# yuki-koyama/sequential-line-search

Hardware: AMD Instinct MI355X
Metric: GP-fit+acq-max step time (ms) and candidate-evals/sec at N=8192 D=64 (higher is better)
Workload: dtype f64

## Files before the change

sequential-line-search_amd/csrc/gemm_f64.hpp:

```cpp
#pragma once
#include <hip/hip_runtime.h>

namespace slsk {

typedef double d4_t __attribute__((ext_vector_type(4)));
typedef double d2_t __attribute__((ext_vector_type(2)));

constexpr int GEMM_BM = 128;
constexpr int GEMM_BN = 128;
constexpr int GEMM_BK = 16;
constexpr int GEMM_THREADS = 256;
constexpr int GEMM_LDS_MC_LD = 144;
constexpr int GEMM_LDS_KC_LD = 18;
constexpr int GEMM_LDS_TILE = 16 * 144;
constexpr int GEMM_LDS_BYTES = 4 * GEMM_LDS_TILE * 8;

struct Acc {
    d4_t v[4][4];
    __device__ __forceinline__ void zero() {
#pragma unroll
        for (int i = 0; i < 4; ++i)
#pragma unroll
            for (int j = 0; j < 4; ++j) v[i][j] = d4_t{0.0, 0.0, 0.0, 0.0};
    }
// ... 10 lines not shown
        const int idx = tid + 256 * i;
        if (!KC) {
            const int k = idx >> 6, m2 = idx & 63;
            s.r[i] = *reinterpret_cast<const d2_t*>(P + (long)(2 * m2) + (long)(k0 + k) * ld);
        } else {
            const int m = idx >> 3, k2 = idx & 7;
            s.r[i] = *reinterpret_cast<const d2_t*>(P + (long)(k0 + 2 * k2) + (long)m * ld);
        }
    }
}

template <bool KC>
__device__ __forceinline__ void stage_store(const Stage& s, double* lds, int tid) {
#pragma unroll
    for (int i = 0; i < 4; ++i) {
        const int idx = tid + 256 * i;
        if (!KC) {
            const int k = idx >> 6, m2 = idx & 63;
            *reinterpret_cast<d2_t*>(lds + k * GEMM_LDS_MC_LD + 2 * m2) = s.r[i];
        } else {
            const int m = idx >> 3, k2 = idx & 7;
            *reinterpret_cast<d2_t*>(lds + m * GEMM_LDS_KC_LD + 2 * k2) = s.r[i];
        }
    }
}

template <bool KC>
__device__ __forceinline__ double frag_read(const double* lds, int mbase, int kk, int lane) {
    if (!KC)
        return lds[(4 * kk + (lane >> 4)) * GEMM_LDS_MC_LD + mbase + (lane & 15)];
    else
        return lds[(mbase + (lane & 15)) * GEMM_LDS_KC_LD + 4 * kk + (lane >> 4)];
}

__device__ __forceinline__ void slab_row_to_lds(const double* g, double* l) {
    __builtin_amdgcn_global_load_lds((const __attribute__((address_space(1))) void*)g, (__attribute__((address_space(3))) void*)l, 16, 0,
                                     0);
}

__device__ __forceinline__ void slab_row_to_lds_sc1(const double* g, double* l) {
    __builtin_amdgcn_global_load_lds((const __attribute__((address_space(1))) void*)g, (__attribute__((address_space(3))) void*)l, 16, 0,
                                     16);
}

__device__ __forceinline__ void slab_row_to_lds_saddr(const double* srow, unsigned lane_off, unsigned lds_byte_addr) {
    asm volatile("s_mov_b32 m0, %2\n\ts_nop 0\n\tglobal_load_lds_dwordx4 %0, %1" ::"v"(lane_off), "s"(srow), "s"(lds_byte_addr)
                 : "memory", "m0");
}

template <int N>
__device__ __forceinline__ void ring_wait_barrier() {
    asm volatile("s_waitcnt vmcnt(%0) lgkmcnt(0)\n\ts_barrier" ::"n"(N) : "memory");
}

template <int NJ, int CUR>
__device__ __forceinline__ void mc_slab(Acc& acc, double (&f0)[4 + NJ], double (&f1)[4 + NJ], const double* Arow, const double* Brow,
                                        long lda, long ldb, unsigned lane_off, unsigned lds_base, const double* lds, int cur_rt,
                                        int nxt_rt, int wave, int wm, int wn, int lane) {
    const int cur_off = CUR < 0 ? cur_rt : CUR * 2 * GEMM_LDS_TILE;
    const int nxt_off = CUR < 0 ? nxt_rt : (1 - CUR) * 2 * GEMM_LDS_TILE;
    auto issue = [&](int l) {
        const int r = l & 3;
        const double* g = l < 4 ? Arow + (long)r * lda : Brow + (long)r * ldb;
        const unsigned d = lds_base + 8u * (unsigned)(nxt_off + (l < 4 ? 0 : GEMM_LDS_TILE) + (4 * wave + r) * GEMM_LDS_MC_LD);
        slab_row_to_lds_saddr(g, lane_off, d);
    };
    auto read = [&](double (&f)[4 + NJ], int bufoff, int kk) {
#pragma unroll
        for (int i = 0; i < 4; ++i) f[i] = frag_read<false>(lds + bufoff, wm + 16 * i, kk, lane);
#pragma unroll
        for (int j = 0; j < NJ; ++j) f[4 + j] = frag_read<false>(lds + bufoff + GEMM_LDS_TILE, wn + 16 * j, kk, lane);
    };
#pragma unroll
    for (int kk = 0; kk < 4; ++kk) {
        double(&f)[4 + NJ] = (kk & 1) ? f1 : f0;
        double(&g)[4 + NJ] = (kk & 1) ? f0 : f1;
#pragma unroll
        for (int i = 0; i < 4; ++i) {
#pragma unroll
            for (int j = 0; j < NJ; ++j) {
                acc.v[i][j] = __builtin_amdgcn_mfma_f64_16x16x4f64(f[4 + j], f[i], acc.v[i][j], 0, 0, 0);
                const int m = (kk * 4 + i) * NJ + j + 1;
                if ((m & 1) == 0 && m <= 16) {
                    __builtin_amdgcn_sched_barrier(0);
                    issue(m / 2 - 1);
                    __builtin_amdgcn_sched_barrier(0);
                }
            }
            if (kk < 3 && i == 2) {
                __builtin_amdgcn_sched_barrier(0);
                read(g, cur_off, kk + 1);
                __builtin_amdgcn_sched_barrier(0);
            }
            if (kk == 3 && i == 1) {
                __builtin_amdgcn_sched_barrier(0);
                ring_wait_barrier<0>();
                read(g, nxt_off, 0);
                __builtin_amdgcn_sched_barrier(0);
            }
        }
    }
}

template <int NJ = 4, bool EVEN = false>
__device__ __forceinline__ void gemm_tile_mc(Acc& acc, const double* __restrict__ A, long lda, const double* __restrict__ B, long ldb,
                                             int kb, int ke, double* lds, int nhalf = 0) {
    if (kb >= ke) return;
    const int tid = threadIdx.x, lane = tid & 63;
    const int wave = __builtin_amdgcn_readfirstlane(tid >> 6);
    const int wm = (wave & 1) * 64;
    const int wn = NJ == 4 ? (wave >> 1) * 64 : 64 * nhalf + (wave >> 1) * 32;
    const unsigned lane_off = 16u * lane;
    const unsigned lds_base = (unsigned)(unsigned long long)(__attribute__((address_space(3))) double*)lds;
    const double* A0 = A + (long)(kb + 4 * wave) * lda;
    const double* B0 = B + (long)(kb + 4 * wave) * ldb;
#pragma unroll
    for (int r = 0; r < 4; ++r) {
        slab_row_to_lds_saddr(A0 + (long)r * lda, lane_off, lds_base + 8u * (unsigned)((4 * wave + r) * GEMM_LDS_MC_LD));
        slab_row_to_lds_saddr(B0 + (long)r * ldb, lane_off, lds_base + 8u * (unsigned)(GEMM_LDS_TILE + (4 * wave + r) * GEMM_LDS_MC_LD));
    }
    ring_wait_barrier<0>();
    double f0[4 + NJ], f1[4 + NJ];
#pragma unroll
    for (int i = 0; i < 4; ++i) f0[i] = frag_read<false>(lds, wm + 16 * i, 0, lane);
#pragma unroll
    for (int j = 0; j < NJ; ++j) f0[4 + j] = frag_read<false>(lds + GEMM_LDS_TILE, wn + 16 * j, 0, lane);
    const int nslab = (ke - kb) / GEMM_BK;
    const double* Arow = A0;
    const double* Brow = B0;
    if constexpr (EVEN) {
        for (int s = 0; s < nslab; s += 2) {
            Arow += (long)GEMM_BK * lda;
            Brow += (long)GEMM_BK * ldb;
            mc_slab<NJ, 0>(acc, f0, f1, Arow, Brow, lda, ldb, lane_off, lds_base, lds, 0, 0, wave, wm, wn, lane);
            const bool last = s + 2 == nslab;
            Arow = last ? A0 : Arow + (long)GEMM_BK * lda;
            Brow = last ? B0 : Brow + (long)GEMM_BK * ldb;
            mc_slab<NJ, 1>(acc, f0, f1, Arow, Brow, lda, ldb, lane_off, lds_base, lds, 0, 0, wave, wm, wn, lane);
        }
    } else {
        int cur = 0;
        for (int s = 0; s < nslab; ++s) {
            const bool last = s + 1 == nslab;
            Arow = last ? A0 : Arow + (long)GEMM_BK * lda;
            Brow = last ? B0 : Brow + (long)GEMM_BK * ldb;
            const int nxt = cur ^ (2 * GEMM_LDS_TILE);
            mc_slab<NJ, -1>(acc, f0, f1, Arow, Brow, lda, ldb, lane_off, lds_base, lds, cur, nxt, wave, wm, wn, lane);
            cur = nxt;
        }
    }
    ring_wait_barrier<0>();
}

template <bool A_KC, bool B_KC, int NJ = 4, bool EVEN = false>
__device__ __forceinline__ void gemm_tile(Acc& acc, const double* __restrict__ A, long lda,
                                          const double* __restrict__ B, long ldb, int kb, int ke, double* lds, int nhalf = 0) {
    if constexpr (!A_KC && !B_KC) {
        gemm_tile_mc<NJ, EVEN>(acc, A, lda, B, ldb, kb, ke, lds, nhalf);
    } else {
        static_assert(NJ == 4, "half tiles exist for the M-contiguous form only");
        const int tid = threadIdx.x;
        const int lane = tid & 63;
        const int wave = tid >> 6;
        const int wm = (wave & 1) * 64;
        const int wn = (wave >> 1) * 64;
        if (kb >= ke) return;
        Stage sa, sb;
        stage_load<A_KC>(sa, A, lda, kb, tid);
        stage_load<B_KC>(sb, B, ldb, kb, tid);
        stage_store<A_KC>(sa, lds, tid);
        stage_store<B_KC>(sb, lds + GEMM_LDS_TILE, tid);
        __syncthreads();
        int cur = 0;
        for (int k0 = kb; k0 < ke; k0 += GEMM_BK) {
            const bool more = (k0 + GEMM_BK) < ke;
            if (more) {
                stage_load<A_KC>(sa, A, lda, k0 + GEMM_BK, tid);
                stage_load<B_KC>(sb, B, ldb, k0 + GEMM_BK, tid);
            }
            const double* la = lds + cur;
            const double* lb = lds + cur + GEMM_LDS_TILE;
#pragma unroll
            for (int kk = 0; kk < 4; ++kk) {
                double af[4], bf[4];
#pragma unroll
                for (int i = 0; i < 4; ++i) af[i] = frag_read<A_KC>(la, wm + 16 * i, kk, lane);
#pragma unroll
                for (int j = 0; j < 4; ++j) bf[j] = frag_read<B_KC>(lb, wn + 16 * j, kk, lane);
#pragma unroll
                for (int i = 0; i < 4; ++i)
#pragma unroll
                    for (int j = 0; j < 4; ++j)
                        acc.v[i][j] = __builtin_amdgcn_mfma_f64_16x16x4f64(bf[j], af[i], acc.v[i][j], 0, 0, 0);
            }
            const int nxt = cur ^ (2 * GEMM_LDS_TILE);
            if (more) {
                stage_store<A_KC>(sa, lds + nxt, tid);
                stage_store<B_KC>(sb, lds + nxt + GEMM_LDS_TILE, tid);
            }
            __syncthreads();
            cur = nxt;
        }
    }
}

constexpr int GEMM_N64_LDS_B = 64 * GEMM_LDS_KC_LD;
constexpr int GEMM_N64_LDS_BUF = GEMM_LDS_TILE + GEMM_N64_LDS_B;
constexpr int GEMM_N64_LDS_BYTES = 2 * GEMM_N64_LDS_BUF * 8;

struct Acc64 {
    d4_t v[2][4];
    __device__ __forceinline__ void zero() {
#pragma unroll
        for (int i = 0; i < 2; ++i)
#pragma unroll
            for (int j = 0; j < 4; ++j) v[i][j] = d4_t{0.0, 0.0, 0.0, 0.0};
    }
};

template <int A_LD>
constexpr int gemm_n64_lds_bytes() {
    return 2 * (16 * A_LD + GEMM_N64_LDS_B) * 8;
}
template <bool A_KC = false, int A_LD = GEMM_LDS_MC_LD>
__device__ __forceinline__ void gemm_tile_n64(Acc64& acc, const double* __restrict__ A, long lda,
                                              const double* __restrict__ B, long ldb, int kb, int ke, double* lds) {
    static_assert(!A_KC || A_LD == GEMM_LDS_MC_LD, "the K-contiguous image has its own padding");
    constexpr int A_SLAB = 16 * A_LD;
    constexpr int BUF = A_SLAB + GEMM_N64_LDS_B;
    const int tid = threadIdx.x;
    const int lane = tid & 63;
    const int wm = (tid >> 6) * 32;
    if (kb >= ke) return;
    Stage sa;
    d2_t sbr[2];
    auto load_b = [&](int k0) {
#pragma unroll
        for (int i = 0; i < 2; ++i) {
            const int idx = tid + 256 * i;
            const int n = idx >> 3, k2 = idx & 7;
            sbr[i] = *reinterpret_cast<const d2_t*>(B + (long)(k0 + 2 * k2) + (long)n * ldb);
        }
    };
    auto store_b = [&](double* l) {
#pragma unroll
        for (int i = 0; i < 2; ++i) {
            const int idx = tid + 256 * i;
            const int n = idx >> 3, k2 = idx & 7;
            *reinterpret_cast<d2_t*>(l + n * GEMM_LDS_KC_LD + 2 * k2) = sbr[i];
        }
    };
    constexpr bool DIRECT_A = !A_KC;
    const int wave_u = __builtin_amdgcn_readfirstlane(tid >> 6);
    auto issue_a = [&](int k0, int bufoff) {
#pragma unroll
        for (int r = 0; r < 4; ++r) {
            const int row = 4 * wave_u + r;
            slab_row_to_lds(A + 2 * lane + (long)(k0 + row) * lda, lds + bufoff + row * A_LD);
        }
    };
    if (DIRECT_A) issue_a(kb, 0);
    else stage_load<A_KC>(sa, A, lda, kb, tid);
    load_b(kb);
    if (DIRECT_A) asm volatile("s_waitcnt vmcnt(0)" ::: "memory");
    else stage_store<A_KC>(sa, lds, tid);
    store_b(lds + A_SLAB);
    __syncthreads();
    int cur = 0;
    for (int k0 = kb; k0 < ke; k0 += GEMM_BK) {
        const bool more = (k0 + GEMM_BK) < ke;
        if (more) {
            if (DIRECT_A) issue_a(k0 + GEMM_BK, cur ^ BUF);
            else stage_load<A_KC>(sa, A, lda, k0 + GEMM_BK, tid);
            load_b(k0 + GEMM_BK);
        }
        const double* la = lds + cur;
        const double* lb = lds + cur + A_SLAB;
#pragma unroll
        for (int kk = 0; kk < 4; ++kk) {
            double af[2], bf[4];
#pragma unroll
            for (int i = 0; i < 2; ++i)
                af[i] = A_KC ? frag_read<true>(la, wm + 16 * i, kk, lane)
                             : la[(4 * kk + (lane >> 4)) * A_LD + wm + 16 * i + (lane & 15)];
#pragma unroll
            for (int j = 0; j < 4; ++j) bf[j] = frag_read<true>(lb, 16 * j, kk, lane);
#pragma unroll
            for (int i = 0; i < 2; ++i)
#pragma unroll
                for (int j = 0; j < 4; ++j)
                    acc.v[i][j] = __builtin_amdgcn_mfma_f64_16x16x4f64(bf[j], af[i], acc.v[i][j], 0, 0, 0);
        }
        const int nxt = cur ^ BUF;
        if (more) {
            if (!DIRECT_A) stage_store<A_KC>(sa, lds + nxt, tid);
            store_b(lds + nxt + A_SLAB);
        }
        if (DIRECT_A) asm volatile("s_waitcnt vmcnt(0)" ::: "memory");
        __syncthreads();
        cur = nxt;
    }
}

__device__ __forceinline__ int acc_m(int i) {
    const int lane = threadIdx.x & 63, wave = threadIdx.x >> 6;
    return (wave & 1) * 64 + 16 * i + (lane & 15);
}
__device__ __forceinline__ int acc_n(int j, int r) {
    const int lane = threadIdx.x & 63, wave = threadIdx.x >> 6;
    return (wave >> 1) * 64 + 16 * j + (lane >> 4) + 4 * r;
}

template <bool HEAVY = false, class F>
__device__ __forceinline__ void acc_tile_by_columns(const Acc& acc, double* lds, F&& f) {
    const int lane = threadIdx.x & 63, wave = __builtin_amdgcn_readfirstlane(threadIdx.x >> 6);
#pragma unroll
    for (int half = 0; half < 2; ++half) {
        __syncthreads();
        if ((wave >> 1) == half) {
#pragma unroll
            for (int i = 0; i < 4; ++i)
#pragma unroll
                for (int j = 0; j < 4; ++j)
#pragma unroll
                    for (int r = 0; r < 4; ++r)
                        lds[(16 * j + (lane >> 4) + 4 * r) * GEMM_LDS_MC_LD + (wave & 1) * 64 + 16 * i + (lane & 15)] = acc.v[i][j][r];
        }
        __syncthreads();
        if constexpr (HEAVY) {
#pragma unroll 2
            for (int q = 0; q < 16; ++q) {
                const int c = wave + 4 * q;
                const d2_t v = *reinterpret_cast<const d2_t*>(lds + c * GEMM_LDS_MC_LD + 2 * lane);
                f(64 * half + c, 2 * lane, v);
            }
        } else {
#pragma unroll
            for (int q = 0; q < 16; ++q) {
                const int c = wave + 4 * q;
                const d2_t v = *reinterpret_cast<const d2_t*>(lds + c * GEMM_LDS_MC_LD + 2 * lane);
                f(64 * half + c, 2 * lane, v);
            }
        }
    }
}

__device__ __forceinline__ int xcd_remap(int b, int nwg) {
    const int q = nwg >> 3, r = nwg & 7;
    const int xcd = b & 7, within = b >> 3;
    const int base = (xcd < r) ? xcd * (q + 1) : r * (q + 1) + (xcd - r) * q;
    return base + within;
}

}
```

sequential-line-search_amd/csrc/kernels_acq.hip:

```cpp
#include <cstdlib>

#include "gemm_f64.hpp"
#include "kernels.hpp"
#include "../../include/sls_hip.h"

namespace slsk {

template <bool MATERN, bool HALF>
__device__ __forceinline__ void acq_tile(int t, int nhalf, int ntm, int ntn, const double* __restrict__ Ks, const double* __restrict__ Cs,
                                         long ldk, const double* __restrict__ Kinv, int Np, double* __restrict__ P,
                                         double* __restrict__ kw_part, double* __restrict__ cw_part, double* lds) {
    const int GM = 8;
    const int gsz = GM * ntn;
    const int g = t / gsz, w = t % gsz;
    const int gm = min(GM, ntm - g * GM);
    const int tm = g * GM + (w % gm), tn = w / gm;
    const int m0 = tm * GEMM_BM, n0 = tn * GEMM_BN;
    Acc acc;
    acc.zero();
    gemm_tile<false, false, HALF ? 2 : 4, true>(acc, Ks + m0, ldk, Kinv + n0, (long)Np, 0, Np, lds, nhalf);
    const int lane = threadIdx.x & 63, wave = threadIdx.x >> 6;
    constexpr int NJ = HALF ? 2 : 4;
    const int nbase = HALF ? 64 * nhalf + (wave >> 1) * 32 : (wave >> 1) * 64;
    double* red = lds;
    double* ex = lds + 1024;
    if (HALF && (wave >> 1) == 1) __syncthreads();
    double skw[4], scw[4];
#pragma unroll
    for (int i = 0; i < 4; ++i) {
        const long gm_ = m0 + acc_m(i);
        double pk = 0.0, pc = 0.0;
        if (HALF && (wave >> 1) == 1) {
            pk = ex[((0 * 2 + (wave & 1)) * 4 + i) * 64 + lane];
            pc = ex[((1 * 2 + (wave & 1)) * 4 + i) * 64 + lane];
        }
        double kv[NJ][4], cv[NJ][4];
#pragma unroll
        for (int j = 0; j < NJ; ++j)
#pragma unroll
            for (int r = 0; r < 4; ++r) {
                const long off = gm_ + (long)(n0 + nbase + 16 * j + (lane >> 4) + 4 * r) * ldk;
                kv[j][r] = Ks[off];
                if (MATERN) cv[j][r] = Cs[off];
            }
#pragma unroll
        for (int j = 0; j < NJ; ++j)
#pragma unroll
            for (int r = 0; r < 4; ++r) {
                const long off = gm_ + (long)(n0 + nbase + 16 * j + (lane >> 4) + 4 * r) * ldk;
                const double wv = acc.v[i][j][r];
                const double k = kv[j][r];
                const double c = MATERN ? cv[j][r] : k;
                const double p = c * wv;
                P[off] = p;
                pc += p;
                if (MATERN) pk += k * wv;
            }
        if (HALF && (wave >> 1) == 0) {
            ex[((0 * 2 + (wave & 1)) * 4 + i) * 64 + lane] = pk;
            ex[((1 * 2 + (wave & 1)) * 4 + i) * 64 + lane] = pc;
        }
        scw[i] = pc;
        skw[i] = MATERN ? pk : pc;
    }
    if (HALF && (wave >> 1) == 0) __syncthreads();
#pragma unroll
    for (int i = 0; i < 4; ++i) {
        skw[i] += __shfl_xor(skw[i], 16);
        skw[i] += __shfl_xor(skw[i], 32);
        scw[i] += __shfl_xor(scw[i], 16);
        scw[i] += __shfl_xor(scw[i], 32);
    }
    if (lane < 16 && (!HALF || (wave >> 1) == 1)) {
#pragma unroll
        for (int i = 0; i < 4; ++i) {
            const int ml = (wave & 1) * 64 + 16 * i + lane;
            const int slot = HALF ? 0 : (wave >> 1);
            red[(slot * 2 + 0) * 128 + ml] = skw[i];
            red[(slot * 2 + 1) * 128 + ml] = scw[i];
        }
    }
    __syncthreads();
    if (threadIdx.x < 128) {
        const int ml = threadIdx.x;
        if (HALF) {
            kw_part[(long)(2 * tn + nhalf) * ldk + m0 + ml] = red[0 * 128 + ml];
            cw_part[(long)(2 * tn + nhalf) * ldk + m0 + ml] = red[1 * 128 + ml];
        } else {
            kw_part[(long)(2 * tn + 0) * ldk + m0 + ml] = red[0 * 128 + ml] + red[2 * 128 + ml];
            cw_part[(long)(2 * tn + 0) * ldk + m0 + ml] = red[1 * 128 + ml] + red[3 * 128 + ml];
        }
    }
}

template <bool MATERN>
__global__ __launch_bounds__(256, 1) void acq_gemm_kernel(const double* __restrict__ Ks, const double* __restrict__ Cs, long ldk,
                                                          int Sp, const double* __restrict__ Kinv, int Np,
                                                          double* __restrict__ P, double* __restrict__ kw_part,
                                                          double* __restrict__ cw_part, int* __restrict__ sync,
                                                          int phase, int ntiles, int prio, int gate_every, int nx) {
    extern __shared__ __attribute__((aligned(16))) char smem[];
    double* lds = reinterpret_cast<double*>(smem);
    const int ntm = Sp / GEMM_BM, ntn = Np / GEMM_BN;
    if (sync == nullptr) {
        acq_tile<MATERN, false>(xcd_remap(blockIdx.x, ntiles), 0, ntm, ntn, Ks, Cs, ldk, Kinv, Np, P, kw_part, cw_part, lds);
        return;
    }
    const int xcd = blockIdx.x % nx, slot = blockIdx.x / nx, slots = gridDim.x / nx;
    const int nchunks = (ntiles + slots - 1) / slots;
    const int half = slots >> 1;
    const int grp = phase > 0 ? (slot >= half ? 1 : 0) : 0;
    if (prio && slot >= half) __builtin_amdgcn_s_setprio(1);
    int* gate = sync + 2 * xcd + grp;
    const int per_gen = phase > 0 ? half : slots;
    if (grp == 1) {
        if (threadIdx.x == 0) {
            const long long t0 = wall_clock64();
            while (wall_clock64() - t0 < phase) __builtin_amdgcn_s_sleep(16);
        }
        __syncthreads();
    }
    int gen = 0;
    for (int c = xcd; c < nchunks; c += nx, ++gen) {
        if (gen > 0 && phase >= 0 && gen % gate_every == 0) {
            if (threadIdx.x == 0) {
                const int target = per_gen * gen;
                const long long t0 = wall_clock64();
                while (__hip_atomic_load(gate, __ATOMIC_RELAXED, __HIP_MEMORY_SCOPE_AGENT) < target &&
                       wall_clock64() - t0 < 20000)
                    __builtin_amdgcn_s_sleep(16);
            }
            __syncthreads();
        }
        const int t = c * slots + slot;
        if (t < ntiles) acq_tile<MATERN, false>(t, 0, ntm, ntn, Ks, Cs, ldk, Kinv, Np, P, kw_part, cw_part, lds);
        __syncthreads();
        if (threadIdx.x == 0) __hip_atomic_fetch_add(gate, 1, __ATOMIC_RELAXED, __HIP_MEMORY_SCOPE_AGENT);
    }
}

template <bool MATERN>
__global__ __launch_bounds__(256, 1) void acq_gemm_half_kernel(const double* __restrict__ Ks, const double* __restrict__ Cs, long ldk,
                                                               int Sp, const double* __restrict__ Kinv, int Np,
                                                               double* __restrict__ P, double* __restrict__ kw_part,
                                                               double* __restrict__ cw_part, int tail_first) {
    extern __shared__ __attribute__((aligned(16))) char smem[];
    double* lds = reinterpret_cast<double*>(smem);
    const int u = xcd_remap(blockIdx.x, gridDim.x);
    acq_tile<MATERN, true>(tail_first + (u >> 1), u & 1, Sp / GEMM_BM, Np / GEMM_BN, Ks, Cs, ldk, Kinv, Np, P, kw_part, cw_part, lds);
}

int launch_acq_gemm(hipStream_t s, const double* Ks, const double* Cs, long ldk, int Sp, const double* Kinv, int Np, double* P,
                    double* kw_part, double* cw_part, int* sync) {
    const int nt = (Sp / GEMM_BM) * (Np / GEMM_BN);
    const int persist_env = (int)tune(TUNE_PERSIST, 1);
    const int phase = (int)tune(TUNE_GATE_PHASE, tune(TUNE_ACQ_WG_PER_CU, 1) == 2 ? 2000 : 0);
    const int gate_every = std::max(1, (int)tune(TUNE_GATE_EVERY, tune(TUNE_ACQ_WG_PER_CU, 1) == 2 ? 1 : 16));
    const int prio = 0;
    const int wg_per_cu = tune(TUNE_ACQ_WG_PER_CU, 1) == 2 ? 2 : 1;
    const ChipGeometry chip = chip_geometry();
    const int cap = chip.n_cu * wg_per_cu;
    const int nx = (chip.n_xcd <= 8 && cap % chip.n_xcd == 0) ? chip.n_xcd : 1;
    const int lds_bytes = wg_per_cu == 1 ? 96 * 1024 : GEMM_LDS_BYTES;
    ensure_dyn_lds((const void*)acq_gemm_kernel<false>, lds_bytes);
    ensure_dyn_lds((const void*)acq_gemm_kernel<true>, lds_bytes);
    ensure_dyn_lds((const void*)acq_gemm_half_kernel<false>, lds_bytes);
    ensure_dyn_lds((const void*)acq_gemm_half_kernel<true>, lds_bytes);
    const bool persist = persist_env && sync && nt >= 2 * cap && Np >= 2048;
    const int phase_k = persist_env == 2 ? -1 : phase;
    const bool tail_ok = tune_on(TUNE_TAIL_SPLIT);
    const int rem = nt % cap;
    const int tail = (tail_ok && rem > 0 && rem <= cap / 2) ? rem : 0;
    const int nmain = nt - tail;
    int* sy = nullptr;
    int grid = nmain;
    if (persist && nmain >= 2 * cap) {
        (void)hipMemsetAsync(sync, 0, 16 * sizeof(int), s);
        sy = sync;
        grid = cap;
    }
    const bool matern = Cs != Ks;
    if (nmain > 0) {
        if (matern)
            hipLaunchKernelGGL(acq_gemm_kernel<true>, dim3(grid), dim3(GEMM_THREADS), lds_bytes, s, Ks, Cs, ldk, Sp, Kinv, Np, P,
                               kw_part, cw_part, sy, phase_k, nmain, prio, gate_every, nx);
        else
            hipLaunchKernelGGL(acq_gemm_kernel<false>, dim3(grid), dim3(GEMM_THREADS), lds_bytes, s, Ks, Cs, ldk, Sp, Kinv, Np, P,
                               kw_part, cw_part, sy, phase_k, nmain, prio, gate_every, nx);
    }
    if (tail > 0) {
        if (matern)
            hipLaunchKernelGGL(acq_gemm_half_kernel<true>, dim3(2 * tail), dim3(GEMM_THREADS), lds_bytes, s, Ks, Cs, ldk, Sp, Kinv,
                               Np, P, kw_part, cw_part, nmain);
        else
            hipLaunchKernelGGL(acq_gemm_half_kernel<false>, dim3(2 * tail), dim3(GEMM_THREADS), lds_bytes, s, Ks, Cs, ldk, Sp, Kinv,
                               Np, P, kw_part, cw_part, nmain);
    }
    return nmain;
}

__device__ __forceinline__ void var_tile(int tm, int tn, const double* __restrict__ Ks, long ldk, const double* __restrict__ Linv,
                                         int Np, double* __restrict__ kw_part, double* __restrict__ cw_part, double* lds) {
    const int m0 = tm * GEMM_BM, n0 = tn * GEMM_BN;
    Acc acc;
    acc.zero();
    gemm_tile<false, false, 4, true>(acc, Ks + m0, ldk, Linv + n0, (long)Np, 0, GEMM_BN * (tn + 1), lds);
    const int lane = threadIdx.x & 63, wave = threadIdx.x >> 6;
    double sv[4];
#pragma unroll
    for (int i = 0; i < 4; ++i) {
        double p = 0.0;
#pragma unroll
        for (int j = 0; j < 4; ++j)
#pragma unroll
            for (int r = 0; r < 4; ++r) p = fma(acc.v[i][j][r], acc.v[i][j][r], p);
        p += __shfl_xor(p, 16);
        p += __shfl_xor(p, 32);
        sv[i] = p;
    }
    __syncthreads();
    double* red = lds;
    if (lane < 16) {
#pragma unroll
        for (int i = 0; i < 4; ++i) red[(wave >> 1) * 128 + (wave & 1) * 64 + 16 * i + lane] = sv[i];
    }
    __syncthreads();
    if (threadIdx.x < 128) {
        const int ml = threadIdx.x;
        kw_part[(long)(2 * tn) * ldk + m0 + ml] = red[ml] + red[128 + ml];
        cw_part[(long)(2 * tn) * ldk + m0 + ml] = 0.0;
    }
    __syncthreads();
}

__global__ __launch_bounds__(256, 2) void var_gemm_kernel(const double* __restrict__ Ks, long ldk, int Sp,
                                                          const double* __restrict__ Linv, int Np,
                                                          double* __restrict__ kw_part, double* __restrict__ cw_part, int pair) {
    extern __shared__ __attribute__((aligned(16))) char smem[];
    double* lds = reinterpret_cast<double*>(smem);
    const int ntm = Sp / GEMM_BM, ntn = Np / GEMM_BN;
    if (!pair) {
        const int T = ntm * ntn;
        int tm = blockIdx.x % ntm, tn = ntn - 1 - blockIdx.x / ntm;
        if ((ntm & 7) == 0 && (ntn & 7) == 0) {
            const int t = xcd_remap(blockIdx.x, T);
            const int per = T >> 3;
            const int x = t / per, l = t - x * per;
            const int gid = (l >> 6) * 8 + x, w = l & 63;
            const int ngm = ntm >> 3;
            tn = ntn - 1 - (8 * (gid / ngm) + (w >> 3));
            tm = 8 * (gid % ngm) + (w & 7);
        }
        var_tile(tm, tn, Ks, ldk, Linv, Np, kw_part, cw_part, lds);
        return;
    }
    const int tm = blockIdx.x % ntm, p = blockIdx.x / ntm;
    const int hi = ntn - 1 - p;
    var_tile(tm, hi, Ks, ldk, Linv, Np, kw_part, cw_part, lds);
    if (p < hi) var_tile(tm, p, Ks, ldk, Linv, Np, kw_part, cw_part, lds);
}

void launch_var_gemm(hipStream_t s, const double* Ks, long ldk, int Sp, const double* Linv, int Np, double* kw_part,
                     double* cw_part) {
    ensure_dyn_lds((const void*)var_gemm_kernel, GEMM_LDS_BYTES);
    const int ntm = Sp / GEMM_BM, ntn = Np / GEMM_BN;
    const int pair = (ntm * ntn < 1024 && ntn > 1) ? 1 : 0;
    const int grid = pair ? ntm * ((ntn + 1) / 2) : ntm * ntn;
    hipLaunchKernelGGL(var_gemm_kernel, dim3(grid), dim3(GEMM_THREADS), GEMM_LDS_BYTES, s, Ks, ldk, Sp, Linv, Np, kw_part, cw_part,
                       pair);
}

__global__ __launch_bounds__(256, 2) void grad_gemm_kernel(const double* __restrict__ P, const double* __restrict__ Cs, long ldk,
                                                           int Sp, const double* __restrict__ XT, const double* __restrict__ XaT,
                                                           long ld, int Np, int Dcols, double* __restrict__ Gs,
                                                           double* __restrict__ Gm) {
    extern __shared__ __attribute__((aligned(16))) char smem[];
    double* lds = reinterpret_cast<double*>(smem);
    const int ntm = Sp / GEMM_BM;
    const int tm = blockIdx.x % ntm, tn = blockIdx.x / ntm;
    const int m0 = tm * GEMM_BM, n0 = tn * GEMM_BN;
    const double* A = blockIdx.y == 0 ? P : Cs;
    const double* B = blockIdx.y == 0 ? XT : XaT;
    double* C = blockIdx.y == 0 ? Gs : Gm;
    Acc acc;
    acc.zero();
    gemm_tile<false, true>(acc, A + m0, ldk, B + (long)n0 * ld, ld, 0, Np, lds);
#pragma unroll
    for (int i = 0; i < 4; ++i)
#pragma unroll
        for (int j = 0; j < 4; ++j)
#pragma unroll
            for (int r = 0; r < 4; ++r) C[(long)(m0 + acc_m(i)) + (long)(n0 + acc_n(j, r)) * ldk] = acc.v[i][j][r];
}

constexpr int GRAD64_A_LD = 136;
__global__ __launch_bounds__(256, 3) void grad_gemm64_kernel(const double* __restrict__ P, const double* __restrict__ Cs, long ldk,
                                                             int Sp, const double* __restrict__ XT, const double* __restrict__ XaT,
                                                             long ld, int Np, double* __restrict__ Gs, double* __restrict__ Gm,
                                                             double* __restrict__ part) {
    extern __shared__ __attribute__((aligned(16))) char smem[];
    double* lds = reinterpret_cast<double*>(smem);
    const int m0 = blockIdx.x * GEMM_BM;
    const double* A = blockIdx.y == 0 ? P : Cs;
    const double* B = blockIdx.y == 0 ? XT : XaT;
    const bool split = gridDim.z > 1;
    double* C = split ? part + ((long)blockIdx.z * 2 + blockIdx.y) * (long)Sp * 64 : (blockIdx.y == 0 ? Gs : Gm);
    const long ldc = split ? (long)Sp : ldk;
    const int q = Np / 4;
    Acc64 tot;
    tot.zero();
    const int c0 = split ? blockIdx.z : 0, c1 = split ? blockIdx.z + 1 : 4;
    for (int c = c0; c < c1; ++c) {
        Acc64 acc;
        acc.zero();
        gemm_tile_n64<false, GRAD64_A_LD>(acc, A + m0, ldk, B, ld, c * q, (c + 1) * q, lds);
#pragma unroll
        for (int i = 0; i < 2; ++i)
#pragma unroll
            for (int j = 0; j < 4; ++j) tot.v[i][j] = (c == c0) ? acc.v[i][j] : tot.v[i][j] + acc.v[i][j];
    }
    const int lane = threadIdx.x & 63, wm = (threadIdx.x >> 6) * 32;
#pragma unroll
    for (int i = 0; i < 2; ++i)
#pragma unroll
        for (int j = 0; j < 4; ++j)
#pragma unroll
            for (int r = 0; r < 4; ++r)
                C[(long)(m0 + wm + 16 * i + (lane & 15)) + (long)(16 * j + (lane >> 4) + 4 * r) * ldc] = tot.v[i][j][r];
}

__global__ __launch_bounds__(256) void grad_reduce4_kernel(const double* __restrict__ part, int Sp, long ldk, double* __restrict__ Gs,
                                                           double* __restrict__ Gm, int passes) {
    const long idx = blockIdx.x * 256L + threadIdx.x;
    if (idx >= (long)Sp * 64) return;
    const long n = idx % Sp, d = idx / Sp;
    const long stride = (long)Sp * 64;
    for (int y = 0; y < passes; ++y) {
        const double* p = part + (long)y * stride + idx;
        const double v = ((p[0] + p[2 * stride]) + p[4 * stride]) + p[6 * stride];
        (y == 0 ? Gs : Gm)[n + d * ldk] = v;
    }
}

void launch_grad_gemm(hipStream_t s, const double* P, const double* Cs, long ldk, int Sp, const double* XT, const double* XaT,
                      long ld, int Np, int Dcols, double* Gs, double* Gm, double* part, int passes) {
    ensure_dyn_lds((const void*)grad_gemm_kernel, GEMM_LDS_BYTES);
    ensure_dyn_lds((const void*)grad_gemm64_kernel, gemm_n64_lds_bytes<GRAD64_A_LD>());
    if (Dcols < 0) {
        const bool split = part != nullptr && grad_gemm_wants_split(Sp);
        hipLaunchKernelGGL(grad_gemm64_kernel, dim3(Sp / GEMM_BM, passes, split ? 4 : 1), dim3(GEMM_THREADS), gemm_n64_lds_bytes<GRAD64_A_LD>(), s, P, Cs,
                           ldk, Sp, XT, XaT, ld, Np, Gs, Gm, part);
        if (split)
            hipLaunchKernelGGL(grad_reduce4_kernel, dim3((unsigned)(((long)Sp * 64 + 255) / 256)), dim3(256), 0, s, part, Sp, ldk, Gs, Gm,
                               passes);
        return;
    }
    const int nt = (Sp / GEMM_BM) * (Dcols / GEMM_BN);
    hipLaunchKernelGGL(grad_gemm_kernel, dim3(nt, passes), dim3(GEMM_THREADS), GEMM_LDS_BYTES, s, P, Cs, ldk, Sp, XT, XaT, ld, Np, Dcols,
                       Gs, Gm);
}

__global__ __launch_bounds__(256) void finalize_kernel(FinalizeArgs p) {
    const int n = blockIdx.x * 256 + threadIdx.x;
    if (n >= p.S) return;
    double mu = 0.0, ca = 0.0, kw = 0.0, cw = 0.0;
    const int tm_ = n >> 7, grp_ = tm_ >> 3;
    const int gm_ = min(8, p.ntm - 8 * grp_);
    const int tile_base = grp_ * 8 * p.nbt + (tm_ - 8 * grp_);
    #pragma unroll 8
    for (int t = 0; t < p.nbt; ++t) {
        mu += p.mu_part[(long)t * p.ldk + n];
        ca += p.ca_part[(long)t * p.ldk + n];
        double kt = p.kw_part[(long)(2 * t) * p.ldk + n], ct = p.cw_part[(long)(2 * t) * p.ldk + n];
        if (tile_base + t * gm_ >= p.split_first) {
            kt += p.kw_part[(long)(2 * t + 1) * p.ldk + n];
            ct += p.cw_part[(long)(2 * t + 1) * p.ldk + n];
        }
        kw += kt;
        cw += ct;
    }
    if (p.kw_solve_part) {
        kw = 0.0;
        for (int t = 0; t < p.nbt; ++t) kw += p.kw_solve_part[(long)(2 * t) * p.ldk + n];
    }
    const double s2 = p.a - kw;
    const double sigma = s2 < 0.0 ? 0.0 : sqrt(s2);
    if (p.mu) p.mu[n] = mu;
    if (p.sigma) p.sigma[n] = sigma;
    const bool need_g = p.dmu || p.dsigma || p.grad;
    double Phi = 0.0, phi = 0.0;
    bool bad = false;
    if (p.val || p.grad) {
        if (p.acq == SLS_ACQ_EXPECTED_IMPROVEMENT) {
            const double diff = mu - p.mu_best;
            const double u = diff / sigma;
            Phi = 0.5 * erfc(-u * 0.70710678118654752440);
            phi = exp(-0.5 * u * u) * 0.39894228040143267794;
            const double ei = diff * Phi + sigma * phi;
            bad = (sigma < 1e-10) || isnan(ei);
            if (p.val) p.val[n] = bad ? 0.0 : ei;
        } else {
            if (p.val) p.val[n] = mu + p.ucb_h * sigma;
        }
    }
    if (!need_g) return;
    const double inv_sigma = 1.0 / sigma;
    if (p.grad && p.acq == SLS_ACQ_EXPECTED_IMPROVEMENT) {
        for (int d = 0; d < p.D && !bad; ++d) {
            const double xt = p.XsT[n + (long)d * p.ldk];
            const double il = p.inv_ell[d];
            const double dm = -il * (xt * ca - p.Gm[n + (long)d * p.ldk]);
            const double ds = inv_sigma * il * (xt * cw - p.Gs[n + (long)d * p.ldk]);
            if (isnan(Phi * dm + phi * ds)) bad = true;
        }
    }
    #pragma unroll 4
    for (int d = 0; d < p.D; ++d) {
        const double xt = p.XsT[n + (long)d * p.ldk];
        const double il = p.inv_ell[d];
        const double dm = -il * (xt * ca - p.Gm[n + (long)d * p.ldk]);
        const double ds = inv_sigma * il * (xt * cw - p.Gs[n + (long)d * p.ldk]);
        if (p.dmu) p.dmu[n + (long)d * p.ldo] = dm;
        if (p.dsigma) p.dsigma[n + (long)d * p.ldo] = ds;
        if (p.grad) {
            double g;
            if (p.acq == SLS_ACQ_EXPECTED_IMPROVEMENT) g = bad ? 0.0 : Phi * dm + phi * ds;
            else g = dm + p.ucb_h * ds;
            p.grad[n + (long)d * p.ldo] = g;
        }
    }
}

void launch_finalize(hipStream_t s, const FinalizeArgs& a) {
    hipLaunchKernelGGL(finalize_kernel, dim3((a.S + 255) / 256), dim3(256), 0, s, a);
}

__global__ __launch_bounds__(256) void combine_kernel(int S, int D, long ld, const double* __restrict__ mu,
                                                     const double* __restrict__ sigma, const double* __restrict__ dmu,
                                                     const double* __restrict__ dsigma, int acq, double mu_best, double ucb_h,
                                                     double* __restrict__ val, double* __restrict__ grad) {
    const int n = blockIdx.x * 256 + threadIdx.x;
    if (n >= S) return;
    const double m = mu[n], sg = sigma[n];
    if (acq == SLS_ACQ_EXPECTED_IMPROVEMENT) {
        const double diff = m - mu_best;
        const double u = diff / sg;
        const double Phi = 0.5 * erfc(-u * 0.70710678118654752440);
        const double phi = exp(-0.5 * u * u) * 0.39894228040143267794;
        const double ei = diff * Phi + sg * phi;
        bool bad = (sg < 1e-10) || isnan(ei);
        val[n] = bad ? 0.0 : ei;
        if (grad) {
            for (int d = 0; d < D && !bad; ++d)
                if (isnan(Phi * dmu[n + d * ld] + phi * dsigma[n + d * ld])) bad = true;
            for (int d = 0; d < D; ++d) grad[n + d * ld] = bad ? 0.0 : Phi * dmu[n + d * ld] + phi * dsigma[n + d * ld];
        }
    } else {
        val[n] = m + ucb_h * sg;
        if (grad)
            for (int d = 0; d < D; ++d) grad[n + d * ld] = dmu[n + d * ld] + ucb_h * dsigma[n + d * ld];
    }
}
void launch_combine(hipStream_t s, int S, int D, long ld, const double* mu, const double* sigma, const double* dmu,
                    const double* dsigma, int acq, double mu_best, double ucb_h, double* val, double* grad) {
    hipLaunchKernelGGL(combine_kernel, dim3((S + 255) / 256), dim3(256), 0, s, S, D, ld, mu, sigma, dmu, dsigma, acq, mu_best,
                       ucb_h, val, grad);
}

__global__ __launch_bounds__(256) void clamp_starts_kernel(const double* __restrict__ starts, int D, int S, double* __restrict__ xt,
                                                           long ld, int Sp) {
    const int n = blockIdx.x * 256 + threadIdx.x;
    if (n >= Sp) return;
    for (int d = 0; d < D; ++d) {
        double v = 0.5;
        if (n < S) {
            v = starts[d + (long)n * D];
            v = v < 0.0 ? 0.0 : (v > 1.0 ? 1.0 : v);
        }
        xt[n + (long)d * ld] = v;
    }
}
void launch_clamp_starts(hipStream_t s, const double* starts, int D, int S, double* xt, long ld, int Sp) {
    hipLaunchKernelGGL(clamp_starts_kernel, dim3((Sp + 255) / 256), dim3(256), 0, s, starts, D, S, xt, ld, Sp);
}

__global__ __launch_bounds__(64) void lbfgs_step_kernel(LbfgsState st, const double* __restrict__ val,
                                                         const double* __restrict__ grad, int first) {
    const int q = threadIdx.x >> 4;
    const int j = blockIdx.x * 16 + (threadIdx.x & 15);
    if (j >= st.nlive) return;
    auto gsum = [](double v) {
        v += __shfl_xor(v, 16);
        v += __shfl_xor(v, 32);
        return v;
    };
    auto gmax = [](double v) {
        v = fmax(v, __shfl_xor(v, 16));
        v = fmax(v, __shfl_xor(v, 32));
        return v;
    };
    const int n = st.live ? st.live[j] : j;
    const long ld = st.ld, ldv = st.ldv;
    const int D = st.D, m = st.m;
    double* __restrict__ x_ = st.x; double* __restrict__ g_ = st.g; double* __restrict__ dir_ = st.dir;
    double* __restrict__ xt_ = st.xt; double* __restrict__ scr_ = st.scr;
    double* __restrict__ ShA = st.Sh; double* __restrict__ YhA = st.Yh;
    double f_v = 0.0, t_v = 1.0;
    int hlen_v = 0, hpos_v = 0, nbt_v = 0;
    bool done = false;
    int idx_new = -1;
    double rho_new = 0.0;
    bool need_dir = false;
    if (first) {
        f_v = -val[j];
        #pragma unroll 4
        for (int d = q; d < D; d += 4) {
            x_[n + d * ld] = xt_[n + d * ld];
            g_[n + d * ld] = -grad[j + d * ldv];
        }
        need_dir = true;
    } else {
        if (st.done[n]) return;
        f_v = st.f[n]; t_v = st.t[n]; hlen_v = st.hlen[n]; hpos_v = st.hpos[n]; nbt_v = st.nbt[n];
        const double ft = -val[j];
        double gs = 0.0, ss = 0.0;
        #pragma unroll 4
        for (int d = q; d < D; d += 4) {
            const double sd = xt_[n + d * ld] - x_[n + d * ld];
            gs += g_[n + d * ld] * sd;
            ss += sd * sd;
        }
        gs = gsum(gs);
        ss = gsum(ss);
        if (ss == 0.0) {
            if (q == 0) st.done[n] = 1;
            return;
        }
        if (ft <= f_v + st.c1 * gs) {
            double sy = 0.0, yy = 0.0, xmoved = 0.0;
            const int idx = hpos_v;
            double* __restrict__ Sh = ShA + (long)idx * D * ld;
            double* __restrict__ Yh = YhA + (long)idx * D * ld;
            #pragma unroll 4
            for (int d = q; d < D; d += 4) {
                const double xtd = xt_[n + d * ld], gtd = -grad[j + d * ldv];
                const double sd = xtd - x_[n + d * ld];
                const double yd = gtd - g_[n + d * ld];
                xmoved += lbfgs_x_moved(x_[n + d * ld], xtd, st.xtol_rel);
                Sh[n + d * ld] = sd;
                Yh[n + d * ld] = yd;
                sy += sd * yd;
                yy += yd * yd;
                x_[n + d * ld] = xtd;
                g_[n + d * ld] = gtd;
            }
            sy = gsum(sy);
            yy = gsum(yy);
            if (sy > 1e-10 * yy && sy > 0.0) {
                idx_new = idx;
                rho_new = 1.0 / sy;
                if (q == 0) st.rho[(long)idx * ld + n] = rho_new;
                hpos_v = (idx + 1) % m;
                if (hlen_v < m) hlen_v += 1;
            }
            if (lbfgs_f_stalled(f_v, ft, st.ftol_rel) || (st.xtol_rel > 0.0 && gsum(xmoved) == 0.0)) done = true;
            f_v = ft;
            need_dir = true;
        } else {
            t_v *= st.shrink;
            nbt_v += 1;
            if (nbt_v > st.max_backtracks) done = true;
        }
    }
    if (!done && need_dir) {
        double pgmax = 0.0, pgn2 = 0.0;
        #pragma unroll 4
        for (int d = q; d < D; d += 4) {
            double v = g_[n + d * ld];
            const double xv = x_[n + d * ld];
            if ((xv <= 0.0 && v > 0.0) || (xv >= 1.0 && v < 0.0)) v = 0.0;
            scr_[n + d * ld] = v;
            dir_[n + d * ld] = v;
            pgmax = fmax(pgmax, fabs(v));
            pgn2 += v * v;
        }
        pgmax = gmax(pgmax);
        pgn2 = gsum(pgn2);
        if (!(pgmax > st.gtol)) {
            done = true;
        } else {
            const int hlen = hlen_v;
            const int hpos = hpos_v;
            auto rho_of = [&](int idx) { return idx == idx_new ? rho_new : st.rho[(long)idx * ld + n]; };
            double al[8];
#pragma unroll
            for (int h = 0; h < 8; ++h) {
                al[h] = 0.0;
                if (h < hlen) {
                    const int idx = (hpos - 1 - h + 2 * m) % m;
                    const double* __restrict__ Sh = ShA + (long)idx * D * ld;
                    const double* __restrict__ Yh = YhA + (long)idx * D * ld;
                    double dot = 0.0;
                    #pragma unroll 4
                    for (int d = q; d < D; d += 4) dot += Sh[n + d * ld] * dir_[n + d * ld];
                    al[h] = rho_of(idx) * gsum(dot);
                    #pragma unroll 4
                    for (int d = q; d < D; d += 4) dir_[n + d * ld] -= al[h] * Yh[n + d * ld];
                }
            }
            double gamma;
            if (hlen > 0) {
                const int idx = (hpos - 1 + m) % m;
                const double* __restrict__ Sh = ShA + (long)idx * D * ld;
                const double* __restrict__ Yh = YhA + (long)idx * D * ld;
                double sy = 0.0, yy = 0.0;
                #pragma unroll 4
                for (int d = q; d < D; d += 4) {
                    sy += Sh[n + d * ld] * Yh[n + d * ld];
                    yy += Yh[n + d * ld] * Yh[n + d * ld];
                }
                gamma = gsum(sy) / gsum(yy);
            } else {
                const double nn = sqrt(pgn2);
                gamma = 1.0 / (nn > 1.0 ? nn : 1.0);
            }
            #pragma unroll 4
            for (int d = q; d < D; d += 4) dir_[n + d * ld] *= gamma;
#pragma unroll
            for (int h = 7; h >= 0; --h) {
                if (h < hlen) {
                    const int idx = (hpos - 1 - h + 2 * m) % m;
                    const double* __restrict__ Sh = ShA + (long)idx * D * ld;
                    const double* __restrict__ Yh = YhA + (long)idx * D * ld;
                    double dot = 0.0;
                    #pragma unroll 4
                    for (int d = q; d < D; d += 4) dot += Yh[n + d * ld] * dir_[n + d * ld];
                    const double beta = rho_of(idx) * gsum(dot);
                    #pragma unroll 4
                    for (int d = q; d < D; d += 4) dir_[n + d * ld] += Sh[n + d * ld] * (al[h] - beta);
                }
            }
            double gd = 0.0;
            #pragma unroll 4
            for (int d = q; d < D; d += 4) {
                const double pg = scr_[n + d * ld];
                const double dv = (pg == 0.0) ? 0.0 : -dir_[n + d * ld];
                dir_[n + d * ld] = dv;
                gd += pg * dv;
            }
            gd = gsum(gd);
            if (!(gd < 0.0)) {
                hlen_v = 0;
                const double nn = sqrt(pgn2);
// ... 440 lines not shown
```

sequential-line-search_amd/csrc/tuning.hpp:

```cpp
#pragma once
#include <atomic>
#include <cstdlib>
#include <mutex>

namespace slsk {
#define SLS_TUNING_KEYS(X)                                                                                                      \
    X(POOL_MB) X(FIT_SMALL) X(TRI_PREDICT) X(WAVE_PATH) X(IO_STAGE) X(EVAL_ZEROCOPY) X(WAVE_TRACE) X(COMPACT) \
    X(NLL_SMALL) X(SMALL_ZEROCOPY) X(NLL_BATCH) X(MAP_DEVICE) X(MAP_TRACE) X(SMALL_XLDS) X(MULTI_RCCL) X(PERSIST)                \
    X(ACQ_WG_PER_CU) X(GATE_PHASE) X(TAIL_SPLIT) X(LBFGS_REG) X(TRI_WG_PER_CU) X(POTRF_MODE) X(POTRF_DNBO) X(POTRF_NBO)          \
    X(LAUUM_N64) X(TRTRI_NARROW) X(POTRI_FUSED) X(POTRF_STREAM) X(POTRF_SPLIT) X(POTRI_W1) X(POTRF_TIMEOUT_TICKS) X(POTRF_DNEAR) X(POTRI_PLAST)  \
    X(POTRI_CX) X(POTRI_CK) X(WAVE_STAGE) X(WAVE_COOP) X(GRAD_SPLIT_TILES) X(EVAL_SLOTS) X(GATE_EVERY) X(POTRF_FUSE_SYRK) X(POTRI_POOL) X(POTRF_POOL) X(POTRI_POOL_KEEP) X(POTRI_POOL_NEAR) X(POTRI_POOL_NEAR_W) X(GRAM_GUARD)
enum TuneKey {
#define SLS_TK(name) TUNE_##name,
    SLS_TUNING_KEYS(SLS_TK)
#undef SLS_TK
    TUNE_COUNT
};
struct SlsTuning {
    std::atomic<long long> word[TUNE_COUNT];
};
namespace tuning_detail {
inline SlsTuning& table() {
    static SlsTuning t;
    return t;
}
inline void parse() {
    static const char* const names[TUNE_COUNT] = {
#define SLS_TK(name) "SLS_" #name,
        SLS_TUNING_KEYS(SLS_TK)
#undef SLS_TK
    };
    SlsTuning& t = table();
    for (int k = 0; k < TUNE_COUNT; ++k) {
        const char* v = getenv(names[k]);
        t.word[k].store(v ? (((long long)atol(v)) << 1) | 1 : 0, std::memory_order_relaxed);
    }
}
}
inline const SlsTuning& tuning() {
    static std::once_flag once;
    std::call_once(once, tuning_detail::parse);
    return tuning_detail::table();
}
inline void tuning_reload() {
    (void)tuning();
    tuning_detail::parse();
}
inline long tune(TuneKey k, long dflt) {
    const long long w = tuning().word[k].load(std::memory_order_relaxed);
    return (w & 1) ? (long)(w >> 1) : dflt;
}
inline bool tune_on(TuneKey k, bool dflt = true) { return tune(k, dflt ? 1 : 0) != 0; }
inline bool tune_set(TuneKey k) { return (tuning().word[k].load(std::memory_order_relaxed) & 1) != 0; }

}
```

Before: 537,800.

## Add hand-scheduled software-pipelined n64 GEMM path for gradient kernel

```diff
diff --git a/sequential-line-search_amd/csrc/gemm_f64.hpp b/sequential-line-search_amd/csrc/gemm_f64.hpp
--- a/sequential-line-search_amd/csrc/gemm_f64.hpp
+++ b/sequential-line-search_amd/csrc/gemm_f64.hpp
@@ -336,6 +336,105 @@
     }
 }
 
+template <int A_LD, int CUR>
+__device__ __forceinline__ void n64_slab(Acc64& acc, double (&f0)[6], double (&f1)[6], d2_t (&sbr)[2], const double* Arow,
+                                         const double* Bnext, long lda, long ldb, unsigned lane_off, unsigned b_lane_off,
+                                         unsigned lds_base, double* lds, int wave, int wm, int lane, int tid) {
+    constexpr int A_SLAB = 16 * A_LD;
+    constexpr int BUF = A_SLAB + GEMM_N64_LDS_B;
+    constexpr int cur_off = CUR * BUF, nxt_off = (1 - CUR) * BUF;
+    auto read = [&](double (&f)[6], int bufoff, int kk) {
+#pragma unroll
+        for (int i = 0; i < 2; ++i) f[i] = lds[bufoff + (4 * kk + (lane >> 4)) * A_LD + wm + 16 * i + (lane & 15)];
+#pragma unroll
+        for (int j = 0; j < 4; ++j) f[2 + j] = frag_read<true>(lds + bufoff + A_SLAB, 16 * j, kk, lane);
+    };
+    __builtin_amdgcn_sched_barrier(0);
+#pragma unroll
+    for (int i = 0; i < 2; ++i) {
+        const int idx = tid + 256 * i;
+        *reinterpret_cast<d2_t*>(lds + nxt_off + A_SLAB + (idx >> 3) * GEMM_LDS_KC_LD + 2 * (idx & 7)) = sbr[i];
+    }
+#pragma unroll
+    for (int i = 0; i < 2; ++i)
+        sbr[i] = *reinterpret_cast<const d2_t*>(reinterpret_cast<const char*>(Bnext + (long)(32 * i) * ldb) + b_lane_off);
+    __builtin_amdgcn_sched_barrier(0);
+#pragma unroll
+    for (int kk = 0; kk < 4; ++kk) {
+        double(&f)[6] = (kk & 1) ? f1 : f0;
+        double(&g)[6] = (kk & 1) ? f0 : f1;
+#pragma unroll
+        for (int i = 0; i < 2; ++i) {
+#pragma unroll
+            for (int j = 0; j < 4; ++j) {
+                acc.v[i][j] = __builtin_amdgcn_mfma_f64_16x16x4f64(f[2 + j], f[i], acc.v[i][j], 0, 0, 0);
+                const int m = (kk * 2 + i) * 4 + j + 1;
+                if ((m & 1) == 0 && m <= 8) {
+                    const int r = m / 2 - 1;
+                    __builtin_amdgcn_sched_barrier(0);
+                    slab_row_to_lds_saddr(Arow + (long)r * lda, lane_off,
+                                          lds_base + 8u * (unsigned)(nxt_off + (4 * wave + r) * A_LD));
+                    __builtin_amdgcn_sched_barrier(0);
+                }
+            }
+            if (i == 0) {
+                __builtin_amdgcn_sched_barrier(0);
+                if (kk < 3) {
+                    read(g, cur_off, kk + 1);
+                } else {
+                    ring_wait_barrier<0>();
+                    read(g, nxt_off, 0);
+                }
+                __builtin_amdgcn_sched_barrier(0);
+            }
+        }
+    }
+}
+
+template <int A_LD>
+__device__ __forceinline__ void gemm_tile_n64s(Acc64& acc, const double* __restrict__ A, long lda, const double* __restrict__ B,
+                                               long ldb, int kb, int ke, double* lds) {
+    constexpr int A_SLAB = 16 * A_LD;
+    if (kb >= ke) return;
+    const int tid = threadIdx.x, lane = tid & 63;
+    const int wave = __builtin_amdgcn_readfirstlane(tid >> 6);
+    const int wm = wave * 32;
+    const unsigned lane_off = 16u * lane;
+    const unsigned b_lane_off = 8u * (unsigned)(2 * (tid & 7) + (long)(tid >> 3) * ldb);
+    const unsigned lds_base = (unsigned)(unsigned long long)(__attribute__((address_space(3))) double*)lds;
+    const double* A0 = A + (long)(kb + 4 * wave) * lda;
+    const double* B0 = B + kb;
+#pragma unroll
+    for (int r = 0; r < 4; ++r) slab_row_to_lds_saddr(A0 + (long)r * lda, lane_off, lds_base + 8u * (unsigned)((4 * wave + r) * A_LD));
+    d2_t sbr[2];
+#pragma unroll
+    for (int i = 0; i < 2; ++i) {
+        const int idx = tid + 256 * i;
+        const d2_t v = *reinterpret_cast<const d2_t*>(reinterpret_cast<const char*>(B0 + (long)(32 * i) * ldb) + b_lane_off);
+        *reinterpret_cast<d2_t*>(lds + A_SLAB + (idx >> 3) * GEMM_LDS_KC_LD + 2 * (idx & 7)) = v;
+        sbr[i] = *reinterpret_cast<const d2_t*>(reinterpret_cast<const char*>(B0 + GEMM_BK + (long)(32 * i) * ldb) + b_lane_off);
+    }
+    ring_wait_barrier<0>();
+    double f0[6], f1[6];
+#pragma unroll
+    for (int i = 0; i < 2; ++i) f0[i] = lds[(lane >> 4) * A_LD + wm + 16 * i + (lane & 15)];
+#pragma unroll
+    for (int j = 0; j < 4; ++j) f0[2 + j] = frag_read<true>(lds + A_SLAB, 16 * j, 0, lane);
+    const int nslab = (ke - kb) / GEMM_BK;
+    const double* Arow = A0;
+    const double* Brow = B0 + GEMM_BK;
+    for (int s = 0; s < nslab; s += 2) {
+        const bool last = s + 2 == nslab;
+        Arow += (long)GEMM_BK * lda;
+        Brow = last ? B0 : Brow + GEMM_BK;
+        n64_slab<A_LD, 0>(acc, f0, f1, sbr, Arow, Brow, lda, ldb, lane_off, b_lane_off, lds_base, lds, wave, wm, lane, tid);
+        Arow = last ? A0 : Arow + (long)GEMM_BK * lda;
+        Brow += GEMM_BK;
+        n64_slab<A_LD, 1>(acc, f0, f1, sbr, Arow, Brow, lda, ldb, lane_off, b_lane_off, lds_base, lds, wave, wm, lane, tid);
+    }
+    ring_wait_barrier<0>();
+}
+
 __device__ __forceinline__ int acc_m(int i) {
     const int lane = threadIdx.x & 63, wave = threadIdx.x >> 6;
     return (wave & 1) * 64 + 16 * i + (lane & 15);
diff --git a/sequential-line-search_amd/csrc/kernels_acq.hip b/sequential-line-search_amd/csrc/kernels_acq.hip
--- a/sequential-line-search_amd/csrc/kernels_acq.hip
+++ b/sequential-line-search_amd/csrc/kernels_acq.hip
@@ -294,6 +294,7 @@
 }
 
 constexpr int GRAD64_A_LD = 136;
+template <bool SCHED>
 __global__ __launch_bounds__(256, 3) void grad_gemm64_kernel(const double* __restrict__ P, const double* __restrict__ Cs, long ldk,
                                                              int Sp, const double* __restrict__ XT, const double* __restrict__ XaT,
                                                              long ld, int Np, double* __restrict__ Gs, double* __restrict__ Gm,
@@ -313,7 +314,8 @@
     for (int c = c0; c < c1; ++c) {
         Acc64 acc;
         acc.zero();
-        gemm_tile_n64<false, GRAD64_A_LD>(acc, A + m0, ldk, B, ld, c * q, (c + 1) * q, lds);
+        if constexpr (SCHED) gemm_tile_n64s<GRAD64_A_LD>(acc, A + m0, ldk, B, ld, c * q, (c + 1) * q, lds);
+        else gemm_tile_n64<false, GRAD64_A_LD>(acc, A + m0, ldk, B, ld, c * q, (c + 1) * q, lds);
 #pragma unroll
         for (int i = 0; i < 2; ++i)
 #pragma unroll
@@ -345,10 +347,12 @@
 void launch_grad_gemm(hipStream_t s, const double* P, const double* Cs, long ldk, int Sp, const double* XT, const double* XaT,
                       long ld, int Np, int Dcols, double* Gs, double* Gm, double* part, int passes) {
     ensure_dyn_lds((const void*)grad_gemm_kernel, GEMM_LDS_BYTES);
-    ensure_dyn_lds((const void*)grad_gemm64_kernel, gemm_n64_lds_bytes<GRAD64_A_LD>());
+    ensure_dyn_lds((const void*)grad_gemm64_kernel<false>, gemm_n64_lds_bytes<GRAD64_A_LD>());
+    ensure_dyn_lds((const void*)grad_gemm64_kernel<true>, gemm_n64_lds_bytes<GRAD64_A_LD>());
     if (Dcols < 0) {
         const bool split = part != nullptr && grad_gemm_wants_split(Sp);
-        hipLaunchKernelGGL(grad_gemm64_kernel, dim3(Sp / GEMM_BM, passes, split ? 4 : 1), dim3(GEMM_THREADS), gemm_n64_lds_bytes<GRAD64_A_LD>(), s, P, Cs,
+        const auto kern = tune_on(TUNE_ROUND_FORMS) ? grad_gemm64_kernel<true> : grad_gemm64_kernel<false>;
+        hipLaunchKernelGGL(kern, dim3(Sp / GEMM_BM, passes, split ? 4 : 1), dim3(GEMM_THREADS), gemm_n64_lds_bytes<GRAD64_A_LD>(), s, P, Cs,
                            ldk, Sp, XT, XaT, ld, Np, Gs, Gm, part);
         if (split)
             hipLaunchKernelGGL(grad_reduce4_kernel, dim3((unsigned)(((long)Sp * 64 + 255) / 256)), dim3(256), 0, s, part, Sp, ldk, Gs, Gm,
diff --git a/sequential-line-search_amd/csrc/tuning.hpp b/sequential-line-search_amd/csrc/tuning.hpp
--- a/sequential-line-search_amd/csrc/tuning.hpp
+++ b/sequential-line-search_amd/csrc/tuning.hpp
@@ -9,7 +9,7 @@
     X(NLL_SMALL) X(SMALL_ZEROCOPY) X(NLL_BATCH) X(MAP_DEVICE) X(MAP_TRACE) X(SMALL_XLDS) X(MULTI_RCCL) X(PERSIST)                \
     X(ACQ_WG_PER_CU) X(GATE_PHASE) X(TAIL_SPLIT) X(LBFGS_REG) X(TRI_WG_PER_CU) X(POTRF_MODE) X(POTRF_DNBO) X(POTRF_NBO)          \
     X(LAUUM_N64) X(TRTRI_NARROW) X(POTRI_FUSED) X(POTRF_STREAM) X(POTRF_SPLIT) X(POTRI_W1) X(POTRF_TIMEOUT_TICKS) X(POTRF_DNEAR) X(POTRI_PLAST)  \
-    X(POTRI_CX) X(POTRI_CK) X(WAVE_STAGE) X(WAVE_COOP) X(GRAD_SPLIT_TILES) X(EVAL_SLOTS) X(GATE_EVERY) X(POTRF_FUSE_SYRK) X(POTRI_POOL) X(POTRF_POOL) X(POTRI_POOL_KEEP) X(POTRI_POOL_NEAR) X(POTRI_POOL_NEAR_W) X(GRAM_GUARD)
+    X(POTRI_CX) X(POTRI_CK) X(WAVE_STAGE) X(WAVE_COOP) X(GRAD_SPLIT_TILES) X(EVAL_SLOTS) X(GATE_EVERY) X(POTRF_FUSE_SYRK) X(POTRI_POOL) X(POTRF_POOL) X(POTRI_POOL_KEEP) X(POTRI_POOL_NEAR) X(POTRI_POOL_NEAR_W) X(GRAM_GUARD) X(ROUND_FORMS)
 enum TuneKey {
 #define SLS_TK(name) TUNE_##name,
     SLS_TUNING_KEYS(SLS_TK)
```

Result: no change. 539,200, median of 6 (+0.3%).
